# mako443/Text2Pos-CVPR2022

Measured on AMD Instinct MI355X. Metric: cells+queries encoded/sec and top-k retrieval QPS, 256-pt cells, 12k-cell DB, higher is better.
Workload: dtype f16x3 (fp32 operands split hi+lo into fp16, 3 f16 MFMAs, fp32 accumulate; fp32-class error) for the encoders / f64 MFMA for the ranking

## Files before the change

include/t2p.h:

```cpp
#ifndef T2P_H
#define T2P_H
#include <stddef.h>
#include <stdint.h>

#ifdef __cplusplus
extern "C" {
#endif

#define T2P_ABI_VERSION 29
#define T2P_DEFAULT_CHUNK_OBJECTS 65000
#define T2P_MAX_CHUNK_OBJECTS 65535
#define T2P_TUNING_MASK 0x1
#define T2P_E_ARG (-1)
#define T2P_E_WORKSPACE (-2)
#define T2P_E_UNSUPPORTED (-3)

typedef void* t2p_stream_t;

int t2p_abi_version(void);
const char* t2p_last_error(void);

typedef struct t2p_cell_weights {
    const float* sa_w1[3];
    const float* sa_b1[3];
    const float* sa_w2[3];
    const float* sa_b2[3];
    const float* ga_w1;
// ... 189 lines not shown
                               float* dx, t2p_stream_t stream);
int t2p_rownorm_backward(const float* x, const float* dy, int64_t n_rows, int32_t dim, float* dx, t2p_stream_t stream);

int t2p_pairwise_ranking(const float* scores, int32_t batch, float margin, float* row_loss, float* d_scores, float* row_count,
                         t2p_stream_t stream);

int t2p_hardest_ranking(const float* scores, int32_t batch, float margin, float* best, int32_t* where, float* d_scores,
                        t2p_stream_t stream);

int t2p_sample_group(const float* xyz, int64_t n_obj, int32_t n_pts, const float* radius_host ,
                     uint8_t* const* fps_idx , uint8_t* const* nbr , uint8_t* const* cnt ,
                     t2p_stream_t stream);
int t2p_group_rows(const float* xyz, int64_t n_obj, int32_t n_pts, const float* radius_host , int32_t self_loops,
                   uint8_t* const* fps_idx , uint16_t* const* rows , uint16_t* const* n_rows ,
                   t2p_stream_t stream);
int t2p_edge_counts(const uint16_t* rows, const uint16_t* n_rows, const int32_t* first_obj, int64_t n_obj, int32_t n_dense,
                    int32_t n_cent, int32_t self_loops, int32_t* counts, t2p_stream_t stream);
int t2p_edge_expand(const uint16_t* rows, const uint16_t* n_rows, const int32_t* first_obj, const int32_t* cent_ptr, int64_t n_obj,
                    int32_t n_dense, int32_t n_cent, int32_t self_loops, int32_t* src, int32_t* dst, t2p_stream_t stream);
int t2p_dedup_rows(const float* xyz, const float* rgb, int64_t n_obj, int32_t n_pts, uint16_t* rows, uint16_t* n_rows,
                   t2p_stream_t stream);
int t2p_knn(const float* x, int32_t dim, const int32_t* seg_ptr, int32_t n_seg, int32_t max_seg_rows, int32_t k,
            int32_t* out_idx, t2p_stream_t stream);
int t2p_gemm(const float* a, int32_t lda, const float* w, const float* bias, float* c, int32_t ldc, int32_t c0,
             int64_t m, int32_t k, int32_t n, int32_t relu, t2p_stream_t stream);
size_t t2p_gemm_tn_workspace_bytes(int64_t m, int32_t k1, int32_t n);
int t2p_gemm_tn(const float* a, int32_t lda, const float* b, int32_t ldb, float* c, int32_t ldc, int64_t m, int32_t k1, int32_t n,
                void* workspace, size_t workspace_bytes, t2p_stream_t stream);
size_t t2p_linear_wgrad_workspace_bytes(int64_t m, int32_t k1, int32_t n);
int t2p_linear_wgrad_f32(const float* dy, int32_t lda, const float* x, int32_t ldb, float* dw, int32_t ldc, float* colsum, int64_t m,
// ... 8 lines not shown
```

text2pos-cvpr2022_amd/_lib.py:

```python
import ctypes as C
import os

import torch

_HERE = os.path.dirname(os.path.abspath(__file__))
LIB_PATH = os.environ.get("T2P_LIB") or os.path.join(_HERE, "libt2p_hip.so")
ABI_VERSION = 29

c_float_p = C.POINTER(C.c_float)
c_void = C.c_void_p


class CellWeights(C.Structure):
    _names = (["sa_w1", "sa_b1", "sa_w2", "sa_b2"], ["ga_w1", "ga_b1", "ga_w2", "ga_b2", "lin1_w", "lin1_b", "lin2_w",
              "lin2_b", "pn_w", "pn_b", "col_w1", "col_b1", "col_w2", "col_b2", "pos_w1", "pos_b1", "pos_w2", "pos_b2",
              "merge_w", "merge_b", "g_wp", "g_bp", "g_wq", "g_w2", "g_b2", "lin_w1", "lin_b1", "lin_w2", "lin_b2"])
    _fields_ = ([(n, c_void * 3) for n in _names[0]] + [(n, c_void) for n in _names[1]] +
                [("sa_w2_x3", c_void * 3), ("ga_w2_x3", c_void), ("sa_b2_x3", c_void * 3), ("sa_w2_scale", C.c_float * 3),
                 ("lin1_x3", c_void), ("lin2_x3", c_void), ("merge_x3", c_void), ("pn_x3", c_void), ("g_wp_x3", c_void),
                 ("g_wq_x3", c_void), ("lin1_scale", C.c_float), ("lin2_scale", C.c_float), ("merge_scale", C.c_float),
                 ("pn_scale", C.c_float), ("g_wp_scale", C.c_float), ("g_wq_scale", C.c_float),
                 ("sa_w1_x3", c_void * 3), ("ga_w1_x3", c_void),
                 ("class_embedding", c_void), ("color_embedding", c_void),
                 ("ga_w1_l1", C.c_float), ("ga_b1_absmax", C.c_float), ("sa_wp_l1", C.c_float * 3),
# ... 73 lines not shown
    "t2p_pack_objects": (C.c_int, [c_void, c_void, c_void, c_void, c_void, C.c_int64, C.c_int32, c_void, c_void, c_void, c_void,
                                   c_void]),
    "t2p_pack_scene_objects": (C.c_int, [c_void, c_void, c_void, c_void, c_void, c_void, c_void, C.c_int64, C.c_int32, c_void, c_void,
                                         c_void, c_void, c_void, c_void]),
    "t2p_match_workspace_bytes": (C.c_size_t, [C.c_int64, C.c_int32, C.c_int32, C.c_int32]),
    "t2p_match": (C.c_int, [c_void, c_void, C.c_int64, C.c_int32, C.c_int32, C.c_int32, C.POINTER(MatchWeights),
                            C.c_int32, C.c_float, c_void, c_void, c_void, c_void, c_void, c_void, c_void, C.c_size_t,
                            c_void]),
    "t2p_profile_enable": (None, [C.c_int]),
    "t2p_profile_report": (C.c_int, [C.c_char_p, C.c_size_t]),
    "t2p_profile_repeat": (None, [C.c_char_p, C.c_int32]),
    "t2p_sample_group": (C.c_int, [c_void, C.c_int64, C.c_int32, c_float_p, C.POINTER(c_void), C.POINTER(c_void),
                                   C.POINTER(c_void), c_void]),
    "t2p_group_rows": (C.c_int, [c_void, C.c_int64, C.c_int32, c_float_p, C.c_int32, C.POINTER(c_void), C.POINTER(c_void),
                                 C.POINTER(c_void), c_void]),
    "t2p_edge_counts": (C.c_int, [c_void, c_void, c_void, C.c_int64, C.c_int32, C.c_int32, C.c_int32, c_void, c_void]),
    "t2p_edge_expand": (C.c_int, [c_void, c_void, c_void, c_void, C.c_int64, C.c_int32, C.c_int32, C.c_int32, c_void, c_void, c_void]),
    "t2p_dedup_rows": (C.c_int, [c_void, c_void, C.c_int64, C.c_int32, c_void, c_void, c_void]),
    "t2p_knn": (C.c_int, [c_void, C.c_int32, c_void, C.c_int32, C.c_int32, C.c_int32, c_void, c_void]),
    "t2p_gemm": (C.c_int, [c_void, C.c_int32, c_void, c_void, c_void, C.c_int32, C.c_int32, C.c_int64, C.c_int32,
                           C.c_int32, C.c_int32, c_void]),
    "t2p_rownorm": (C.c_int, [c_void, C.c_int64, C.c_int32, c_void, c_void]),
    "t2p_linear_wgrad_workspace_bytes": (C.c_size_t, [C.c_int64, C.c_int32, C.c_int32]),
    "t2p_linear_wgrad_f32": (C.c_int, [c_void, C.c_int32, c_void, C.c_int32, c_void, C.c_int32, c_void, C.c_int64, C.c_int32,
                                       C.c_int32, c_void, C.c_size_t, c_void]),
    "t2p_gemm_tn_workspace_bytes": (C.c_size_t, [C.c_int64, C.c_int32, C.c_int32]),
    "t2p_gemm_tn": (C.c_int, [c_void, C.c_int32, c_void, C.c_int32, c_void, C.c_int32, C.c_int64, C.c_int32, C.c_int32, c_void,
                              C.c_size_t, c_void]),
}

# ... 29 lines not shown
```

text2pos-cvpr2022_amd/csrc/api.hip:

```cpp
#include <stdarg.h>
#include <stdlib.h>
#include <string.h>

#include <mutex>
#include <set>
#include <utility>

#include "../../include/t2p.h"
#include "t2p_common.h"

namespace t2p {

static thread_local char g_err[512] = "";

void set_error(const char* fmt, ...) {
    va_list ap;
    va_start(ap, fmt);
    vsnprintf(g_err, sizeof(g_err), fmt, ap);
    va_end(ap);
}

int num_cus() {
    static int cached = 0;
    if (cached == 0) {
// ... 249 lines not shown
            gt.B[l] = lds_btab[l] ? nullptr : ws.B[l];
            gt.wp[l] = W.sa_w1[l] + (size_t)cf * Geo::H[l];
            gt.H[l] = Geo::H[l];
            gt.tail[l] = ws.F[l];
            gt.ld_tail[l] = Geo::LD[l];
            gt.tail_col0[l] = Geo::C[l];
        }
        gt.tail_rows[2] = g.gp;
        gt.A1 = sa1_points ? nullptr : ws.A[0];
        gt.w1 = W.sa_w1[0];
        gt.b1 = W.sa_b1[0];
        gt.rgb = rgb;
        gt.H1 = Geo::H[0];
        gt.guard = guard;

        T2P_TRY(launch_sample_group(xyz, n, cfg.n_pts, cfg.radius, gt, st));
        if (!(cfg.tuning & 1) && cfg.n_pts == 256)
            T2P_TRY(launch_dedup_rows(xyz, rgb, n, cfg.n_pts, gt.rows[0], gt.n_rows[0], g.nc[0], st));
        SaParams bp[3] = {};
        for (int l = 0; l < 3; l++) {
            bp[l].n_rows = gt.n_rows[l];
            bp[l].n_obj = n;
            bp[l].prefix_ws = ws.prefix[l];
            bp[l].bounds_ws = ws.bounds[l];
            bp[l].W_x3 = cfg.precision == 1 ? W.sa_w2_x3[l] : nullptr;
            bp[l].wp = lds_btab[l] ? W.sa_w1[l] : nullptr;
            bp[l].n_dense = g.nd[l];
            bp[l].n_cent = g.nc[l];
        }
        bp[0].w1 = sa1_points ? W.sa_w1[0] : nullptr;
        T2P_TRY(launch_sa_balance_levels(bp, Geo::H, Geo::C, st));
    }

    for (int l = 0; l < 3; l++) {
        const int H = Geo::H[l], C = Geo::C[l];
        const int cf = l == 0 ? 3 : Geo::C[l - 1];
        const float* pos_src = l == 0 ? xyz : ws.F[l - 1];
        const int ld_pos = l == 0 ? 3 : Geo::LD[l - 1];
        const int pos_col0 = l == 0 ? 0 : Geo::C[l - 1];
        if (l != 0) {
            WsParams p{};
            p.A = ws.F[l - 1];
            p.lda = Geo::LD[l - 1];
            p.k_live = Geo::C[l - 1] + 4;
            p.W = W.sa_w1[l];
// ... 678 lines not shown
    T2P_CHECK_ARG(xyz && radius_host && fps_idx && rows && n_rows, "group_rows: NULL argument");
    Geo g(n_pts);
    GroupTables gt{};
    gt.self_loops = self_loops ? 1 : 0;
    for (int l = 0; l < 3; l++) {
        T2P_CHECK_ARG(fps_idx[l] && rows[l] && n_rows[l], "group_rows: NULL table of level %d", l);
        gt.fps_idx[l] = fps_idx[l];
        gt.rows[l] = rows[l];
        gt.n_rows[l] = n_rows[l];
        gt.n_dense[l] = g.nd[l];
        gt.n_cent[l] = g.nc[l];
    }
    return launch_sample_group(xyz, n_obj, n_pts, radius_host, gt, (hipStream_t)stream);
}

int t2p_edge_counts(const uint16_t* rows, const uint16_t* n_rows, const int32_t* first_obj, int64_t n_obj, int32_t n_dense,
                    int32_t n_cent, int32_t self_loops, int32_t* counts, t2p_stream_t stream) {
    T2P_CHECK_ARG(n_obj >= 0 && (n_obj == 0 || (rows && n_rows && first_obj && counts)), "edge_counts: NULL argument");
    return launch_edge_counts(rows, n_rows, first_obj, n_obj, n_dense, n_cent, self_loops, counts, (hipStream_t)stream);
}

int t2p_edge_expand(const uint16_t* rows, const uint16_t* n_rows, const int32_t* first_obj, const int32_t* cent_ptr, int64_t n_obj,
                    int32_t n_dense, int32_t n_cent, int32_t self_loops, int32_t* src, int32_t* dst, t2p_stream_t stream) {
    T2P_CHECK_ARG(n_obj >= 0 && (n_obj == 0 || (rows && n_rows && first_obj && cent_ptr)), "edge_expand: NULL argument");
    return launch_edge_expand(rows, n_rows, first_obj, cent_ptr, n_obj, n_dense, n_cent, self_loops, src, dst, (hipStream_t)stream);
}

int t2p_pack_objects(const float* raw_xyz, const float* raw_rgb, const int32_t* obj_ptr, const int32_t* sample_idx,
                     const float* rot_cos_sin, int64_t n_obj, int32_t n_pts, float* xyz, float* rgb, float* center, float* mean_rgb,
                     t2p_stream_t stream) {
// ... 55 lines not shown
```

text2pos-cvpr2022_amd/csrc/sa_rows.hip:

```cpp
#ifndef T2P_RABL
#define T2P_RABL 0
#endif
#include "t2p_common.h"

namespace t2p {
int launch_sa_balance(const SaParams& p, int tile_rows, int n_wg, hipStream_t st);

namespace {

typedef _Float16 half8 __attribute__((ext_vector_type(8)));
typedef __fp16 fp16x2 __attribute__((ext_vector_type(2)));
typedef __attribute__((address_space(3))) void lds_void;
typedef const __attribute__((address_space(1))) void gl_void;

#define MFMA16(a, b, c) __builtin_amdgcn_mfma_f32_32x32x16_f16(a, b, c, 0, 0, 0)
#ifndef T2P_ROWS_AGPR
#define T2P_ROWS_AGPR 1
#endif
#ifndef T2P_ROWS_DIRECT
#define T2P_ROWS_DIRECT 1
#endif
__device__ __forceinline__ constexpr int rows_load_slot(int s, int c) {
    if (s == 0) return c == 0 || c == 4 ? -1 : 10 + (c < 4 ? c - 1 : c - 2);
    if (s == 1) return c == 1 ? 16 : (c == 3 ? 17 : -1);
// ... 31 lines not shown

template <int K, int N, int NC, int NW>
struct RowsCfg {
    static constexpr int NT = 64 * NW;
    static constexpr int ND = 2 * NC;
    static constexpr int S16 = K / 16, NTW = N / 32;
    static constexpr int SLOTS = K / 32;
    static constexpr int SLOT_BYTES = 32 * 128;
    static constexpr int RING_BYTES = SLOTS * SLOT_BYTES;
    static constexpr int MAXR = NC * 33;
    static constexpr int ROWS_CHUNKS = (MAXR * 2 + 1023) / 1024;
    static constexpr int ROWS_BUF = ROWS_CHUNKS * 1024;
    static constexpr int BT_STRIDE = K * 4 + 16;
    static constexpr int CPOS_BUF = 3 * NC * 4;
    static constexpr int ACC_OFF = 0;
    static constexpr int BT_OFF = ACC_OFF + NC * N * 4;
    static constexpr int ROWS_OFF = BT_OFF + NC * BT_STRIDE;
    static constexpr int CPOS_OFF = ROWS_OFF + 3 * ROWS_BUF;
    static constexpr int NR_OFF = CPOS_OFF + 2 * CPOS_BUF;
    static constexpr int SB_OFF = NR_OFF + kSubR * 2;
    static constexpr int DSTL_OFF = SB_OFF + kSubR * 4;
    static constexpr int RING_OFF = (DSTL_OFF + NW * 64 + 1023) / 1024 * 1024;
    static constexpr size_t lds_bytes() { return (size_t)RING_OFF + (T2P_ROWS_DIRECT ? (size_t)0 : (size_t)NW * RING_BYTES); }
    static_assert(K % 32 == 0 && N % 32 == 0 && NC % 64 == 0 && (NC * N / 4) % NT == 0, "shape");
    static_assert(SLOTS == 4, "the counted waits below assume four ring slots per tile (K = 128)");
};

template <int SEL>
__device__ __forceinline__ float sub_half_r(float v, fp16x2 h) {
    float r;
    if constexpr (SEL == 0)
        asm("v_fma_mix_f32 %0, %1, -1.0, %2 op_sel:[0,0,0] op_sel_hi:[1,0,0]" : "=v"(r) : "v"(h), "v"(v));
    else
        asm("v_fma_mix_f32 %0, %1, -1.0, %2 op_sel:[1,0,0] op_sel_hi:[1,0,0]" : "=v"(r) : "v"(h), "v"(v));
    return r;
}

__device__ __forceinline__ void lds_barrier_r() { asm volatile("s_waitcnt lgkmcnt(0)\n\ts_barrier" ::: "memory"); }
__device__ __forceinline__ void wait_ring() { asm volatile("s_waitcnt vmcnt(8)" ::: "memory"); }
__device__ __forceinline__ void wait_all_vm() { asm volatile("s_waitcnt vmcnt(0)" ::: "memory"); }
// ... 50 lines not shown

    uint32_t rd[2][2];
#pragma unroll
    for (int par = 0; par < 2; par++)
#pragma unroll
        for (int j = 0; j < 2; j++)
            rd[par][j] = ringb + (uint32_t)(rr * 128 + (((4 * par + 2 * h + j) ^ ((rr >> 1) & 7)) * 16));
    uint32_t dma_sel[4], dma_chunk[4];
#pragma unroll
    for (int q = 0; q < 4; q++) {
        const int r = 8 * q + (lane >> 3);
        dma_sel[q] = (uint32_t)(r * 4);
        dma_chunk[q] = (uint32_t)((((lane & 7) ^ ((r >> 1) & 7))) * 16);
    }

    for (int i = tid; i < NC * N; i += C::NT) acc_lds[i] = (int)0xFF800000;
    int gtop = 0;

    const int g_begin = p.bounds_ws[blockIdx.x], g_end = p.bounds_ws[blockIdx.x + 1];

    auto dma16 = [&](const void* base, uint32_t voff, uint32_t lds_off) {
        __builtin_amdgcn_global_load_lds((gl_void*)((const char*)base + voff), (lds_void*)(lds + lds_off), 16, 0, 0);
    };
    auto dma_rows = [&](int g) {
        const char* src = (const char*)(p.rows + (int64_t)g * C::MAXR);
        const uint32_t dst = (uint32_t)(C::ROWS_OFF + (g % 3) * C::ROWS_BUF);
#pragma unroll
        for (int c = 0; c < C::ROWS_CHUNKS; c++) {
            if (c % NW != wave) continue;
            uint32_t off = (uint32_t)(c * 1024 + lane * 16);
            if (off + 16 > (uint32_t)(C::MAXR * 2)) off = 0;
// ... 54 lines not shown
#pragma unroll
            for (int q = 0; q < 4; q++) dma_piece(voff, u, q);
        };
#if T2P_ROWS_DIRECT
        constexpr int AHEAD = 5;
        const uint32_t hoff = (uint32_t)(h * 32);
        auto load_half = [&](uint32_t roff, int s_, int j, f32x4 (&x)[2]) {
            if constexpr (!(T2P_RABL & 1)) x[j] = *(const f32x4*)((const char*)p.A + (size_t)roff + (size_t)(s_ * 64 + j * 16));
        };
        auto load_step = [&](uint32_t roff, int s_, f32x4 (&x)[2]) {
            load_half(roff, s_, 0, x);
            load_half(roff, s_, 1, x);
        };
#endif

        auto flush = [&](int g) {
            float* o = p.out + (int64_t)g * NC * (int64_t)p.ldo;
            int top = gtop;
            static_assert(C::NT % (N / 4) == 0, "a thread keeps its column quad over the drain");
#pragma unroll
            for (int k = 0; k < NC * N / 4 / C::NT; k++) {
                const int i = tid + k * C::NT;
                const int c = i / (N / 4), c4 = i % (N / 4);
                typedef int i32x4 __attribute__((ext_vector_type(4)));
                f32x4* a = (f32x4*)(acc_lds + c * N + c4 * 4);
                const f32x4 raw = *a;
                f32x4 v;
#pragma unroll
                for (int e = 0; e < 4; e++) {
                    const float r = fmaxf(raw[e] + bias4[e], 0.f);
                    const int bits = __float_as_int(r);
                    top = bits > top ? bits : top;
                    v[e] = r * p.out_scale;
                }
// ... 26 lines not shown
        lds_barrier_r();

        bool cur_fetched = false;
        uint32_t m_cur = 0;
#if T2P_ROWS_DIRECT
        uint32_t roff_cur = 0;
        f32x4 xw[C::S16][2];
#pragma unroll
        for (int s0 = 0; s0 < C::S16; s0++) xw[s0][0] = xw[s0][1] = f32x4{0.f, 0.f, 0.f, 0.f};
#endif

        for (int gi = 0; gi < cnt; gi++) {
            const int n_g = rows_of(gi), n_g1 = gi + 1 < cnt ? rows_of(gi + 1) : 0;
            const uint32_t sb_g = (uint32_t)__builtin_amdgcn_readfirstlane(sbase[gi]);
            const uint32_t sb_g1 = gi + 1 < cnt ? (uint32_t)__builtin_amdgcn_readfirstlane(sbase[gi + 1]) : 0u;
            int r0 = wave * 32;
            bool have = r0 < n_g;
            const bool did_tile = have;
            half8 a_hi, a_lo;
            f32x16 acc[C::NTW];
            bool pend = false;
            uint2 fourp[4] = {};
            auto read_step = [&](int s, uint32_t brow_, f32x4 (&x)[2], f32x4 (&b)[2]) {
#if T2P_ROWS_DIRECT
#pragma unroll
                for (int j = 0; j < 2; j++) {
                    x[j] = xw[s][j];
                    b[j] = *(const f32x4*)(lds + brow_ + s * 64 + j * 16);
                }
#else
// ... 31 lines not shown
                    m_cur = tile_meta(gi, r0, n_g);
#if T2P_ROWS_DIRECT
                    roff_cur = row_byte(gi, sb_g, m_cur) + hoff;
#pragma unroll
                    for (int s0 = 0; s0 < AHEAD; s0++) load_step(roff_cur, s0, xw[s0]);
#else
                    uint32_t v0[4];
                    tile_voff(row_byte(gi, sb_g, m_cur), v0);
#pragma unroll
                    for (int u = 0; u < C::SLOTS; u++) issue_slot(v0, u);
#endif
                }
                {
                    if constexpr (!T2P_ROWS_DIRECT) wait_ring();
                    f32x4 x[2], b[2];
                    read_step(0, (uint32_t)C::BT_OFF + ((m_cur >> 8) & 127u) * (uint32_t)C::BT_STRIDE + (uint32_t)(h * 32), x, b);
                    uint32_t nh[4], nl[4];
#pragma unroll
                    for (int pr = 0; pr < 4; pr++) {
                        float v[2];
                        prep_a(pr, x, b, v);
                        prep_b(v, nh[pr], nl[pr]);
                    }
                    a_hi = __builtin_bit_cast(half8, u32x4{nh[0], nh[1], nh[2], nh[3]});
                    a_lo = __builtin_bit_cast(half8, u32x4{nl[0], nl[1], nl[2], nl[3]});
                }
            }
            while (have) {
                const bool chain = r0 + NW * 32 < n_g;
                const bool nxt_ok = chain || (gi + 1 < cnt && wave * 32 < n_g1);
                const int gi_n = chain ? gi : (nxt_ok ? gi + 1 : gi);
                const int r0_n = chain ? r0 + NW * 32 : (nxt_ok ? wave * 32 : r0);
                const int n_n = (chain || !nxt_ok) ? n_g : n_g1;
                const uint32_t sb_n = (chain || !nxt_ok) ? sb_g : sb_g1;
                uint32_t m_nxt = tile_meta(gi_n, r0_n, n_n);
                uint32_t vn[4];
#if T2P_ROWS_DIRECT
                uint32_t roff_n = roff_cur;
                (void)vn;
#endif
                const uint32_t dl = (m_cur >> 8) & 127u;
                const uint32_t brow = (uint32_t)C::BT_OFF + dl * (uint32_t)C::BT_STRIDE + (uint32_t)(h * 32);
                asm volatile("ds_write_b16 %0, %1" ::"v"(dstl_addr + (uint32_t)(rr * 2)), "v"(dl * (uint32_t)(N * 4)) : "memory");
                uint2 four[4];

                uint32_t brow_n = 0;

#pragma unroll
                for (int s = 0; s < C::S16 - 1; s++) {
                    f32x4 x[2], b[2];
                    if (!T2P_ROWS_DIRECT && ((s + 1) & 1) == 0) wait_ring();
                    read_step(s + 1, brow, x, b);
                    if (s == C::S16 - 2) {
                        const uint32_t a4 = dstl_addr + (uint32_t)(h * 8);
                        asm volatile("ds_read_b64 %0, %4\n\tds_read_b64 %1, %4 offset:16\n\tds_read_b64 %2, %4 offset:32\n\t"
                                     "ds_read_b64 %3, %4 offset:48"
                                     : "=&v"(four[0]), "=&v"(four[1]), "=&v"(four[2]), "=&v"(four[3]) : "v"(a4) : "memory");
// ... 15 lines not shown
                    SB();
                    uint32_t nh[4], nl[4];
                    float v[2];
                    uint32_t rowbyte_n = 0;
#pragma unroll
                    for (int c = 0; c < 8; c++) {
                        if ((c & 1) == 0) prep_a(c >> 1, x, b, v);
                        else prep_b(v, nh[c >> 1], nl[c >> 1]);
                        if (s == 0) {
                            if (c == 2) rowbyte_n = row_byte(gi_n, sb_n, m_nxt);
#if T2P_ROWS_DIRECT
                            if (c == 4) roff_n = rowbyte_n + hoff;
#else
                            if (c == 4) tile_voff(rowbyte_n, vn);
#endif
                            if (c == 6) brow_n = (uint32_t)C::BT_OFF + ((m_nxt >> 8) & 127u) * (uint32_t)C::BT_STRIDE + (uint32_t)(h * 32);
                        }
#if T2P_ROWS_DIRECT
                        {
                            const int ld = rows_load_slot(s, c);
                            if (ld >= 0) load_half(ld < 2 * C::S16 ? roff_cur : roff_n, (ld >> 1) % C::S16, ld & 1, xw[(ld >> 1) % C::S16]);
                        }
#else
                        if ((s & 1) && (c & 1)) dma_piece(vn, s >> 1, c >> 1);
#endif
                        if (c < 4) mfma_w(acc[c], a_hi, w_lo[c][s], w_in_agpr(true, s), false);
                        else mfma_w(acc[c - 4], a_lo, w_hi[c - 4][s], w_in_agpr(false, s), false);
                        SB();
                    }
                    a_hi = __builtin_bit_cast(half8, u32x4{nh[0], nh[1], nh[2], nh[3]});
                    a_lo = __builtin_bit_cast(half8, u32x4{nl[0], nl[1], nl[2], nl[3]});
// ... 48 lines not shown
                            asm volatile(DS_MAX_STR ::"v"(ad[e]), "a"(acc[C::NTW - 1][e]), "n"((C::NTW - 1) * 128) : "memory");
                        pend = false;
                    }
                }
                have = chain;
                r0 = r0_n;
                cur_fetched = nxt_ok;
                m_cur = m_nxt;
#if T2P_ROWS_DIRECT
                roff_cur = roff_n;
#endif
            }
            if (!did_tile) cur_fetched = false;
            if (!did_tile) wait_all_vm();
            if constexpr (!(T2P_RABL & 16)) lds_barrier_r();
            if constexpr (!(T2P_RABL & 4)) flush(ga + gi);
            if (gi + 1 < cnt) {
                if constexpr (!(T2P_RABL & 4)) build_b(ga + gi + 1);
                if (gi + 3 < cnt) dma_rows(ga + gi + 3);
                if (gi + 2 < cnt) dma_cpos(ga + gi + 2);
            }
            if constexpr (!(T2P_RABL & 16)) lds_barrier_r();
        }
    }
    wait_all_vm();
    uint32_t gbits = 0;
    guard_track_bits(gbits, gtop);
    if (p.amax_out != nullptr && lane == 0 && gbits != 0u)
        atomicMax(p.amax_out, __float_as_uint(__uint_as_float(gbits) * p.out_scale));
}

// ... 39 lines not shown
```

text2pos-cvpr2022_amd/csrc/sample_group.hip:

```cpp
#include "t2p_common.h"

namespace t2p {

#pragma clang fp contract(off)

namespace {

#ifndef T2P_FPS_PK
#define T2P_FPS_PK 1
#endif

constexpr int kMaxPts = 256;
constexpr int kMaxNbr = 32;

__device__ __forceinline__ float dist2(float ax, float ay, float az, float bx, float by, float bz) {
#pragma clang fp contract(off)
    float dx = ax - bx, dy = ay - by, dz = az - bz;
    float xx = dx * dx, yy = dy * dy, zz = dz * dz;
    float s = xx + yy;
    return s + zz;
}

template <int CTRL>
__device__ __forceinline__ int dpp_i(int v) {
// ... 93 lines not shown
            if (nbr_lds) cnt_lds[c] = (uint8_t)kept;
            if (self_loops && rows_out) rows_out[base + kept] = (uint16_t)(((c | 0x80) << 8) | c);
        }
        base += kept + (self_loops ? 1 : 0);
        if (c + 1 < n_c) {
            const float mx = wave_max_f(bd);
            const unsigned long long tie = __ballot(bd == mx);
            cur = __builtin_amdgcn_readlane(bi, (int)__builtin_ctzll(tie));
        }
    }
    if (rows_out && lane < 4 && base + lane < n_c * (kMaxNbr + 1)) rows_out[base + lane] = 0xFFFF;
    *n_rows_out = base;
    __syncthreads();
}

template <int PPL>
__device__ void level_fast(const float* px, const float* py, const float* pz, int n_c, float r2, uint8_t* sel, float* qx,
                           float* qy, float* qz, uint16_t* __restrict__ rows_out, int self_loops, int* n_rows_out) {
    const int lane = threadIdx.x;
    const int i0 = lane * PPL;
    float x[PPL], y[PPL], z[PPL];
    uint32_t mind[PPL];
#pragma unroll
    for (int j = 0; j < PPL; j++) {
        x[j] = px[i0 + j];
        y[j] = py[i0 + j];
        z[j] = pz[i0 + j];
        mind[j] = 0x7f800000u;
    }
    int cur = 0;
    int base = 0;
    for (int c = 0; c < n_c; c++) {
        const float cx = px[cur], cy = py[cur], cz = pz[cur];
        if (lane == 0) {
            sel[c] = (uint8_t)cur;
            qx[c] = cx;
            qy[c] = cy;
            qz[c] = cz;
        }
        float d[PPL];
        unsigned long long m[PPL];
        if constexpr (T2P_FPS_PK && PPL % 2 == 0) {
            typedef float f32x2 __attribute__((ext_vector_type(2)));
            const f32x2 c2x = {cx, cx}, c2y = {cy, cy}, c2z = {cz, cz};
#pragma unroll
            for (int j = 0; j < PPL; j += 2) {
#pragma clang fp contract(off)
                const f32x2 dx = f32x2{x[j], x[j + 1]} - c2x, dy = f32x2{y[j], y[j + 1]} - c2y, dz = f32x2{z[j], z[j + 1]} - c2z;
                const f32x2 xx = dx * dx, yy = dy * dy, zz = dz * dz;
                const f32x2 sxy = xx + yy;
                const f32x2 dd = sxy + zz;
                d[j] = dd[0];
                d[j + 1] = dd[1];
// ... 5 lines not shown
            }
        } else {
#pragma unroll
            for (int j = 0; j < PPL; j++) {
                d[j] = dist2(x[j], y[j], z[j], cx, cy, cz);
                mind[j] = min(mind[j], __float_as_uint(d[j]));
                m[j] = __ballot(d[j] < r2);
            }
        }
        int lower = 0, count = 0;
#pragma unroll
        for (int j = 0; j < PPL; j++) {
            lower = __builtin_amdgcn_mbcnt_hi((uint32_t)(m[j] >> 32), __builtin_amdgcn_mbcnt_lo((uint32_t)m[j], lower));
            count += __popcll(m[j]);
        }
        const uint32_t tag = (uint32_t)c << 8;
        char* const rows_b = (char*)rows_out;
        if (count <= kMaxNbr) {
            uint32_t off = 2u * (uint32_t)(base + lower);
#pragma unroll
            for (int j = 0; j < PPL; j++) {
                const bool hit = d[j] < r2;
                if (hit) *(uint16_t*)(rows_b + off) = (uint16_t)(tag | (uint32_t)(i0 + j));
                off += hit ? 2u : 0u;
            }
        } else {
            uint32_t pos = (uint32_t)lower;
#pragma unroll
            for (int j = 0; j < PPL; j++) {
                const bool hit = d[j] < r2;
                if (hit && pos < (uint32_t)kMaxNbr) *(uint16_t*)(rows_b + 2u * ((uint32_t)base + pos)) = (uint16_t)(tag | (uint32_t)(i0 + j));
// ... 125 lines not shown
                            {p3, p3 + kMaxPts / 8, p3 + kMaxPts / 4}};
        const float rr[3] = {r0 * r0, r1 * r1, r2 * r2};
#pragma unroll
        for (int l = 0; l < 3; l++) {
            const int n_d = gt.n_dense[l], n_c = gt.n_cent[l];
            if (want_nbr) {
                for (int i = lane; i < n_c * kMaxNbr / 4; i += 64) ((uint32_t*)nbr_lds)[i] = 0u;
            }
            __syncthreads();
            int n_rows = 0;
            uint16_t* g_rows16 = gt.rows[l] ? gt.rows[l] + o * (int64_t)(n_c * (kMaxNbr + 1)) : nullptr;
            if constexpr (FAST) {
                if (l == 0)
                    level_fast<4>(pin[l][0], pin[l][1], pin[l][2], n_c, rr[l], sel_lds, pin[l + 1][0], pin[l + 1][1],
                                  pin[l + 1][2], g_rows16, gt.self_loops, &n_rows);
                else if (l == 1)
                    level_fast<2>(pin[l][0], pin[l][1], pin[l][2], n_c, rr[l], sel_lds, pin[l + 1][0], pin[l + 1][1],
                                  pin[l + 1][2], g_rows16, gt.self_loops, &n_rows);
                else
                    level_fast<1>(pin[l][0], pin[l][1], pin[l][2], n_c, rr[l], sel_lds, pin[l + 1][0], pin[l + 1][1],
                                  pin[l + 1][2], g_rows16, gt.self_loops, &n_rows);
            } else if (n_d > 128)
                level<4>(pin[l][0], pin[l][1], pin[l][2], n_d, n_c, rr[l], sel_lds, pin[l + 1][0], pin[l + 1][1],
                         pin[l + 1][2], nbr_lds, cnt_lds, g_rows16, gt.self_loops, &n_rows);
            else if (n_d > 64)
                level<2>(pin[l][0], pin[l][1], pin[l][2], n_d, n_c, rr[l], sel_lds, pin[l + 1][0], pin[l + 1][1],
                         pin[l + 1][2], nbr_lds, cnt_lds, g_rows16, gt.self_loops, &n_rows);
            else
                level<1>(pin[l][0], pin[l][1], pin[l][2], n_d, n_c, rr[l], sel_lds, pin[l + 1][0], pin[l + 1][1],
                         pin[l + 1][2], nbr_lds, cnt_lds, g_rows16, gt.self_loops, &n_rows);
// ... 149 lines not shown
```

text2pos-cvpr2022_amd/csrc/t2p_common.h:

```cpp
#pragma once
#include <hip/hip_runtime.h>
#include <stdint.h>
#include <stdio.h>

namespace t2p {

void set_error(const char* fmt, ...);

#define T2P_E_ARG (-1)
#define T2P_E_WORKSPACE (-2)
#define T2P_E_UNSUPPORTED (-3)

#define T2P_CHECK_ARG(cond, ...)                  \
    do {                                          \
        if (!(cond)) {                            \
            ::t2p::set_error(__VA_ARGS__);        \
            return T2P_E_ARG;                     \
        }                                         \
    } while (0)

#define T2P_CHECK_LAUNCH(name)                                                   \
    do {                                                                         \
        hipError_t e__ = hipGetLastError();                                      \
        if (e__ != hipSuccess) {                                                 \
// ... 100 lines not shown
    ~ProfScope();
    int slot;
    hipStream_t st;
    void* ev_end;
    int reps;
};
#define T2P_REPEAT(ps) for (int rep_ = (ps).reps; rep_ > 0; --rep_)

struct GroupTables {
    uint8_t* fps_idx[3];
    uint8_t* nbr[3];
    uint8_t* cnt[3];
    uint16_t* rows[3];
    uint16_t* n_rows[3];
    int self_loops;
    int n_dense[3];
    int n_cent[3];
    float* B[3];
    const float* wp[3];
    int H[3];
    float* tail[3];
    int ld_tail[3], tail_col0[3];
    int tail_rows[3];
    float* A1;
    const float* w1;
    const float* b1;
    const float* rgb;
    int H1;
    uint32_t* guard;
};
// ... 90 lines not shown
    int ld_pos, pos_col0;
    const float* feat_src;
    const float* w1;
    const float* b1;
    int n_dense, n_cent;
    int64_t n_obj;
    int32_t* prefix_ws;
    int32_t* bounds_ws;
    int balanced;
    uint32_t* amax_out;
    int out_rows;
};
int launch_ws_sa(int H, int C, const SaParams& p, hipStream_t st);
int launch_sa_x3(int H, int C, const SaParams& p, hipStream_t st);
int sa_x3_launch_shape(int H, int C, int64_t n_obj, int* tile_rows, int* n_wg);
bool sa_rows_selected(int H, int C, const SaParams& p);
int launch_sa_rows(int H, int C, const SaParams& p, hipStream_t st);
int sa_rows_launch_shape(int64_t n_obj, int* tile_rows, int* n_wg);
bool sa_points_selected(int H, int C, const SaParams& p);
int launch_sa_points(int H, int C, const SaParams& p, hipStream_t st);
int sa_points_launch_shape(int64_t n_obj, int* tile_rows, int* n_wg);
bool sa3_selected(int H, int C, const SaParams& p);
int launch_sa3(const SaParams& p, hipStream_t st);
int sa3_launch_shape(int64_t n_obj, int* tile_rows, int* n_wg);
int launch_sa_balance_levels(const SaParams p[3], const int H[3], const int C[3], hipStream_t st);

int launch_bilstm_impl(const float* gate_table , const float* whh ,
                       const void* whh_x3 ,
                       float whh_scale, const int32_t* tokens , const int32_t* lengths, int B, int T, int V, int D,
                       float* hdir_ws , float* out ,
                       hipStream_t st);

int launch_lstm_cell_fwd(const float* pre, const float* table, const int32_t* tokens, const int32_t* lengths, int64_t B, int T,
                         int D, int step, int reverse, const float* c_prev, const float* h_prev, float* gates, float* c,
                         float* h, hipStream_t st);
int launch_lstm_cell_bwd(const float* dh_gemm, const float* dh_carry_in, const float* dc_in, const float* gates,
                         const float* c_prev, const float* c, const int32_t* lengths, int64_t B, int D, int step, float* d_pre,
                         float* dc_out, float* dh_carry_out, hipStream_t st);

// ... 31 lines not shown
```

text2pos-cvpr2022_amd/ops.py:

```python
import ctypes as C
import os
from typing import Dict, Optional

import numpy as np
import torch

from . import _lib as L

_workspaces: Dict[tuple, torch.Tensor] = {}


def _stream(device) -> C.c_void_p:
    return C.c_void_p(torch.cuda.current_stream(device).cuda_stream)


def _ptr(t: Optional[torch.Tensor]) -> C.c_void_p:
    return C.c_void_p(0 if t is None else t.data_ptr())


def _need(t: torch.Tensor, name: str, dtype, ndim=None, device=None):
    if not isinstance(t, torch.Tensor):
        raise RuntimeError(f"{name}: expected a torch.Tensor, got {type(t).__name__}")
    if not t.is_cuda:
        raise RuntimeError(f"{name}: must live on the GPU (got device {t.device}); there is no CPU path")
# ... 159 lines not shown
        counts = torch.empty((n_obj * ncs[l],), dtype=torch.int32, device=dev)
        L.check(L.lib().t2p_edge_counts(_ptr(rows[l]), _ptr(n_rows[l]), _ptr(first_obj), n_obj, nds[l], ncs[l],
                                        int(bool(self_loops)), _ptr(counts), st), "t2p_edge_counts")
        cp = torch.zeros((n_obj * ncs[l] + 1,), dtype=torch.int32, device=dev)
        torch.cumsum(counts, 0, dtype=torch.int32, out=cp[1:])
        cent_ptrs.append(cp)
    totals = torch.stack([cp[-1] for cp in cent_ptrs]).cpu().tolist()
    out = []
    for l in range(3):
        e = int(totals[l])
        src = torch.empty((e,), dtype=torch.int32, device=dev)
        dst = torch.empty((e,), dtype=torch.int32, device=dev)
        L.check(L.lib().t2p_edge_expand(_ptr(rows[l]), _ptr(n_rows[l]), _ptr(first_obj), _ptr(cent_ptrs[l]), n_obj, nds[l], ncs[l],
                                        int(bool(self_loops)), _ptr(src), _ptr(dst), st), "t2p_edge_expand")
        out.append(dict(fps_idx=fps[l], src=src, dst=dst, cent_ptr=cent_ptrs[l], n_dense=nds[l], n_cent=ncs[l]))
    return out


def dedup_rows(xyz: torch.Tensor, rgb: torch.Tensor, rows: torch.Tensor, n_rows: torch.Tensor):
    _need(xyz, "xyz", torch.float32, 3)
    _need(rgb, "rgb", torch.float32, 3, xyz.device)
    _need(rows, "rows", torch.int16, 2, xyz.device)
    _need(n_rows, "n_rows", torch.int16, 1, xyz.device)
    n_obj, n_pts = xyz.shape[0], xyz.shape[1]
    if rows.shape[0] != n_obj or rows.shape[1] != ((n_pts + 1) // 2) * 33 or n_rows.numel() != n_obj:
        raise RuntimeError("dedup_rows: inconsistent shapes")
    L.check(L.lib().t2p_dedup_rows(_ptr(xyz), _ptr(rgb), n_obj, n_pts, _ptr(rows), _ptr(n_rows), _stream(xyz.device)),
            "t2p_dedup_rows")


# ... 564 lines not shown
```

Baseline: 154,100.

## Share neighbour rows of repeated FPS tail centroids at SA level 2

Once farthest-point sampling runs out of distinct points, it keeps returning index 0. At SA level 2 the grouping now writes that repeated tail centroid's neighbour rows only once, under a shared slot code. The row-GEMM kernel max-reduces those rows into an extra accumulator row, then broadcasts it into every tail centroid at flush time, so duplicate neighbour rows are no longer computed. This adds one LDS accumulator row and a ballot-and-merge step to each flush, and it only applies to 256-point objects when the rows kernel is selected.

```diff
diff --git a/include/t2p.h b/include/t2p.h
--- a/include/t2p.h
+++ b/include/t2p.h
@@ -7,10 +7,10 @@
 extern "C" {
 #endif
 
-#define T2P_ABI_VERSION 29
+#define T2P_ABI_VERSION 30
 #define T2P_DEFAULT_CHUNK_OBJECTS 65000
 #define T2P_MAX_CHUNK_OBJECTS 65535
-#define T2P_TUNING_MASK 0x1
+#define T2P_TUNING_MASK 0x5
 #define T2P_E_ARG (-1)
 #define T2P_E_WORKSPACE (-2)
 #define T2P_E_UNSUPPORTED (-3)
@@ -230,6 +230,9 @@
 int t2p_group_rows(const float* xyz, int64_t n_obj, int32_t n_pts, const float* radius_host , int32_t self_loops,
                    uint8_t* const* fps_idx , uint16_t* const* rows , uint16_t* const* n_rows ,
                    t2p_stream_t stream);
+int t2p_group_rows_shared(const float* xyz, int64_t n_obj, int32_t n_pts, const float* radius_host , int32_t self_loops,
+                          int32_t share_mask, uint8_t* const* fps_idx , uint16_t* const* rows ,
+                          uint16_t* const* n_rows , t2p_stream_t stream);
 int t2p_edge_counts(const uint16_t* rows, const uint16_t* n_rows, const int32_t* first_obj, int64_t n_obj, int32_t n_dense,
                     int32_t n_cent, int32_t self_loops, int32_t* counts, t2p_stream_t stream);
 int t2p_edge_expand(const uint16_t* rows, const uint16_t* n_rows, const int32_t* first_obj, const int32_t* cent_ptr, int64_t n_obj,
diff --git a/profiles/tail_rows_census.py b/profiles/tail_rows_census.py
--- /dev/null
+++ b/profiles/tail_rows_census.py
@@ -0,0 +1,89 @@
+#!/usr/bin/env python
+import argparse
+import os
+import sys
+
+import numpy as np
+
+sys.path.insert(0, os.path.join(os.path.dirname(os.path.abspath(__file__)), ".."))
+
+RADII = (0.2, 0.3, 0.4)
+MAX_NBR = 32
+
+
+def level(pos: np.ndarray, r: float):
+    n_d = pos.shape[0]
+    n_c = (n_d + 1) // 2
+    r2 = np.float32(r) * np.float32(r)
+    mind = np.full(n_d, np.inf, dtype=np.float32)
+    fps = np.zeros(n_c, dtype=np.int64)
+    cnt = np.zeros(n_c, dtype=np.int64)
+    cur = 0
+    for c in range(n_c):
+        fps[c] = cur
+        d = pos - pos[cur]
+        d2 = (d[:, 0] * d[:, 0] + d[:, 1] * d[:, 1]) + d[:, 2] * d[:, 2]
+        cnt[c] = min(int((d2 < r2).sum()), MAX_NBR)
+        mind = np.minimum(mind, d2)
+        cur = int(np.argmax(mind))
+    return fps, cnt
+
+
+def dedup_hits(pos: np.ndarray, rgb: np.ndarray, fps: np.ndarray, r: float) -> int:
+    key = np.concatenate([pos, rgb], axis=1).view(np.uint32)
+    _, first = np.unique(key, axis=0, return_index=True)
+    orig = np.zeros(pos.shape[0], dtype=bool)
+    orig[first] = True
+    r2 = np.float32(r) * np.float32(r)
+    kept = 0
+    for c in fps:
+        d = pos - pos[c]
+        d2 = (d[:, 0] * d[:, 0] + d[:, 1] * d[:, 1]) + d[:, 2] * d[:, 2]
+        hits = np.flatnonzero(d2 < r2)[:MAX_NBR]
+        kept += int(orig[hits].sum())
+    return kept
+
+
+def main():
+    ap = argparse.ArgumentParser(description=__doc__.split("\n")[0])
+    ap.add_argument("--seed", type=int, default=20220002, help="bench.py's object stream")
+    ap.add_argument("--objects", type=int, default=3000)
+    args = ap.parse_args()
+    from importlib import import_module
+    S = import_module("text2pos-cvpr2022_amd.synthetic")
+    xyz, rgb, _, _ = S.make_objects(args.seed, 0, args.objects)
+    n = xyz.shape[0]
+    rows = np.zeros(3)
+    rows_dedup = 0.0
+    with_tail = np.zeros(3)
+    tail_cent = np.zeros(3)
+    tail_rows = np.zeros(3)
+    executed = np.zeros(3)
+    cents = np.zeros(3)
+    for o in range(n):
+        pos = xyz[o].astype(np.float32)
+        for l in range(3):
+            fps, cnt = level(pos, RADII[l])
+            n_c = fps.shape[0]
+            tail = (fps == 0) & (np.arange(n_c) > 0)
+            all_rows = cnt.sum() + n_c
+            t_rows = cnt[tail].sum()
+            rows[l] += all_rows
+            cents[l] += n_c
+            with_tail[l] += tail.any()
+            tail_cent[l] += tail.sum()
+            tail_rows[l] += t_rows
+            executed[l] += all_rows - t_rows + (cnt[0] if tail.any() else 0)
+            if l == 0:
+                rows_dedup += dedup_hits(pos, rgb[o].astype(np.float32), fps, RADII[0]) + n_c
+            pos = pos[fps]
+    print(f"{n} objects of seed {args.seed}")
+    print("level | rows/object | objects with a tail | tail centroids | tail rows (non-self) | rows/object, tail shared")
+    for l in range(3):
+        extra = f" ({rows_dedup / n:.0f} after point dedup)" if l == 0 else ""
+        print(f"SA{l + 1}   | {rows[l] / n:8.0f}{extra} | {100 * with_tail[l] / n:5.1f} % | {100 * tail_cent[l] / cents[l]:5.1f} % | "
+              f"{100 * tail_rows[l] / rows[l]:5.1f} % | {executed[l] / n:8.0f} ({100 * (executed[l] / rows[l] - 1):+.1f} %)")
+
+
+if __name__ == "__main__":
+    main()
diff --git a/text2pos-cvpr2022_amd/_lib.py b/text2pos-cvpr2022_amd/_lib.py
--- a/text2pos-cvpr2022_amd/_lib.py
+++ b/text2pos-cvpr2022_amd/_lib.py
@@ -5,7 +5,7 @@
 
 _HERE = os.path.dirname(os.path.abspath(__file__))
 LIB_PATH = os.environ.get("T2P_LIB") or os.path.join(_HERE, "libt2p_hip.so")
-ABI_VERSION = 29
+ABI_VERSION = 30
 
 c_float_p = C.POINTER(C.c_float)
 c_void = C.c_void_p
@@ -111,6 +111,8 @@
                                    C.POINTER(c_void), c_void]),
     "t2p_group_rows": (C.c_int, [c_void, C.c_int64, C.c_int32, c_float_p, C.c_int32, C.POINTER(c_void), C.POINTER(c_void),
                                  C.POINTER(c_void), c_void]),
+    "t2p_group_rows_shared": (C.c_int, [c_void, C.c_int64, C.c_int32, c_float_p, C.c_int32, C.c_int32, C.POINTER(c_void),
+                                        C.POINTER(c_void), C.POINTER(c_void), c_void]),
     "t2p_edge_counts": (C.c_int, [c_void, c_void, c_void, C.c_int64, C.c_int32, C.c_int32, C.c_int32, c_void, c_void]),
     "t2p_edge_expand": (C.c_int, [c_void, c_void, c_void, c_void, C.c_int64, C.c_int32, C.c_int32, C.c_int32, c_void, c_void, c_void]),
     "t2p_dedup_rows": (C.c_int, [c_void, c_void, C.c_int64, C.c_int32, c_void, c_void, c_void]),
diff --git a/text2pos-cvpr2022_amd/csrc/api.hip b/text2pos-cvpr2022_amd/csrc/api.hip
--- a/text2pos-cvpr2022_amd/csrc/api.hip
+++ b/text2pos-cvpr2022_amd/csrc/api.hip
@@ -287,9 +287,6 @@
         gt.H1 = Geo::H[0];
         gt.guard = guard;
 
-        T2P_TRY(launch_sample_group(xyz, n, cfg.n_pts, cfg.radius, gt, st));
-        if (!(cfg.tuning & 1) && cfg.n_pts == 256)
-            T2P_TRY(launch_dedup_rows(xyz, rgb, n, cfg.n_pts, gt.rows[0], gt.n_rows[0], g.nc[0], st));
         SaParams bp[3] = {};
         for (int l = 0; l < 3; l++) {
             bp[l].n_rows = gt.n_rows[l];
@@ -302,6 +299,11 @@
             bp[l].n_cent = g.nc[l];
         }
         bp[0].w1 = sa1_points ? W.sa_w1[0] : nullptr;
+        for (int l = 0; l < 3; l++) gt.share_tail[l] = sa_shares_tail_rows(l, Geo::H[l], Geo::C[l], bp[l], cfg.n_pts, cfg.tuning) ? 1 : 0;
+
+        T2P_TRY(launch_sample_group(xyz, n, cfg.n_pts, cfg.radius, gt, st));
+        if (!(cfg.tuning & 1) && cfg.n_pts == 256)
+            T2P_TRY(launch_dedup_rows(xyz, rgb, n, cfg.n_pts, gt.rows[0], gt.n_rows[0], g.nc[0], st));
         T2P_TRY(launch_sa_balance_levels(bp, Geo::H, Geo::C, st));
     }
 
@@ -1010,6 +1012,27 @@
     return launch_sample_group(xyz, n_obj, n_pts, radius_host, gt, (hipStream_t)stream);
 }
 
+int t2p_group_rows_shared(const float* xyz, int64_t n_obj, int32_t n_pts, const float* radius_host, int32_t self_loops,
+                          int32_t share_mask, uint8_t* const* fps_idx, uint16_t* const* rows, uint16_t* const* n_rows,
+                          t2p_stream_t stream) {
+    T2P_CHECK_ARG(xyz && radius_host && fps_idx && rows && n_rows, "group_rows_shared: NULL argument");
+    T2P_CHECK_ARG((share_mask & ~2) == 0, "group_rows_shared: share_mask=%#x (bit 1: SA level 2; no other level has a shared form)", share_mask);
+    T2P_CHECK_ARG(share_mask == 0 || n_pts == 256, "group_rows_shared: shared lists exist for 256 points per object (n_pts = %d)", n_pts);
+    Geo g(n_pts);
+    GroupTables gt{};
+    gt.self_loops = self_loops ? 1 : 0;
+    for (int l = 0; l < 3; l++) {
+        T2P_CHECK_ARG(fps_idx[l] && rows[l] && n_rows[l], "group_rows_shared: NULL table of level %d", l);
+        gt.fps_idx[l] = fps_idx[l];
+        gt.rows[l] = rows[l];
+        gt.n_rows[l] = n_rows[l];
+        gt.n_dense[l] = g.nd[l];
+        gt.n_cent[l] = g.nc[l];
+        gt.share_tail[l] = (share_mask >> l) & 1;
+    }
+    return launch_sample_group(xyz, n_obj, n_pts, radius_host, gt, (hipStream_t)stream);
+}
+
 int t2p_edge_counts(const uint16_t* rows, const uint16_t* n_rows, const int32_t* first_obj, int64_t n_obj, int32_t n_dense,
                     int32_t n_cent, int32_t self_loops, int32_t* counts, t2p_stream_t stream) {
     T2P_CHECK_ARG(n_obj >= 0 && (n_obj == 0 || (rows && n_rows && first_obj && counts)), "edge_counts: NULL argument");
diff --git a/text2pos-cvpr2022_amd/csrc/sa_rows.hip b/text2pos-cvpr2022_amd/csrc/sa_rows.hip
--- a/text2pos-cvpr2022_amd/csrc/sa_rows.hip
+++ b/text2pos-cvpr2022_amd/csrc/sa_rows.hip
@@ -69,7 +69,8 @@
     static constexpr int BT_STRIDE = K * 4 + 16;
     static constexpr int CPOS_BUF = 3 * NC * 4;
     static constexpr int ACC_OFF = 0;
-    static constexpr int BT_OFF = ACC_OFF + NC * N * 4;
+    static constexpr int XROW = kSaTailCode;
+    static constexpr int BT_OFF = ACC_OFF + (NC + 1) * N * 4;
     static constexpr int ROWS_OFF = BT_OFF + NC * BT_STRIDE;
     static constexpr int CPOS_OFF = ROWS_OFF + 3 * ROWS_BUF;
     static constexpr int NR_OFF = CPOS_OFF + 2 * CPOS_BUF;
@@ -79,6 +80,7 @@
     static constexpr size_t lds_bytes() { return (size_t)RING_OFF + (T2P_ROWS_DIRECT ? (size_t)0 : (size_t)NW * RING_BYTES); }
     static_assert(K % 32 == 0 && N % 32 == 0 && NC % 64 == 0 && (NC * N / 4) % NT == 0, "shape");
     static_assert(SLOTS == 4, "the counted waits below assume four ring slots per tile (K = 128)");
+    static_assert(XROW == NC && (NC & (NC - 1)) == 0 && XROW * N * 4 <= 0xFFFF && XROW < 128, "shared tail slot");
 };
 
 template <int SEL>
@@ -159,7 +161,7 @@
         dma_chunk[q] = (uint32_t)((((lane & 7) ^ ((r >> 1) & 7))) * 16);
     }
 
-    for (int i = tid; i < NC * N; i += C::NT) acc_lds[i] = (int)0xFF800000;
+    for (int i = tid; i < (NC + 1) * N; i += C::NT) acc_lds[i] = (int)0xFF800000;
     int gtop = 0;
 
     const int g_begin = p.bounds_ws[blockIdx.x], g_end = p.bounds_ws[blockIdx.x + 1];
@@ -244,10 +246,26 @@
         };
 #endif
 
-        auto flush = [&](int g) {
+        auto flush = [&](int g, int t0) {
             float* o = p.out + (int64_t)g * NC * (int64_t)p.ldo;
             int top = gtop;
             static_assert(C::NT % (N / 4) == 0, "a thread keeps its column quad over the drain");
+            if (t0 < NC) {
+                f32x4* const ax = (f32x4*)(acc_lds + C::XROW * N + (tid % (N / 4)) * 4);
+                const f32x4 xq = *ax;
+#pragma unroll 1
+                for (int c = tid / (N / 4); c < NC; c += C::NT / (N / 4)) {
+                    if (c < t0) continue;
+                    f32x4* a = (f32x4*)(acc_lds + c * N + (tid % (N / 4)) * 4);
+                    f32x4 r = *a;
+#pragma unroll
+                    for (int e = 0; e < 4; e++) r[e] = fmaxf(r[e], xq[e]);
+                    *a = r;
+                }
+                lds_barrier_r();
+                typedef int i32x4 __attribute__((ext_vector_type(4)));
+                if (tid < N / 4) *(i32x4*)ax = i32x4{(int)0xFF800000, (int)0xFF800000, (int)0xFF800000, (int)0xFF800000};
+            }
 #pragma unroll
             for (int k = 0; k < NC * N / 4 / C::NT; k++) {
                 const int i = tid + k * C::NT;
@@ -304,6 +322,14 @@
             const int n_g = rows_of(gi), n_g1 = gi + 1 < cnt ? rows_of(gi + 1) : 0;
             const uint32_t sb_g = (uint32_t)__builtin_amdgcn_readfirstlane(sbase[gi]);
             const uint32_t sb_g1 = gi + 1 < cnt ? (uint32_t)__builtin_amdgcn_readfirstlane(sbase[gi + 1]) : 0u;
+            int t0;
+            {
+                static_assert(NC == 64, "one lane per centroid");
+                const uint32_t* cp = (const uint32_t*)(lds + C::CPOS_OFF + ((ga + gi) & 1) * C::CPOS_BUF);
+                const bool same = lane > 0 && cp[lane] == cp[0] && cp[NC + lane] == cp[NC] && cp[2 * NC + lane] == cp[2 * NC];
+                const unsigned long long tm = __ballot(same);
+                t0 = tm ? (int)__builtin_ctzll(tm) : NC;
+            }
             int r0 = wave * 32;
             bool have = r0 < n_g;
             const bool did_tile = have;
@@ -365,7 +391,7 @@
                 {
                     if constexpr (!T2P_ROWS_DIRECT) wait_ring();
                     f32x4 x[2], b[2];
-                    read_step(0, (uint32_t)C::BT_OFF + ((m_cur >> 8) & 127u) * (uint32_t)C::BT_STRIDE + (uint32_t)(h * 32), x, b);
+                    read_step(0, (uint32_t)C::BT_OFF + ((m_cur >> 8) & (uint32_t)(NC - 1)) * (uint32_t)C::BT_STRIDE + (uint32_t)(h * 32), x, b);
                     uint32_t nh[4], nl[4];
 #pragma unroll
                     for (int pr = 0; pr < 4; pr++) {
@@ -391,7 +417,7 @@
                 (void)vn;
 #endif
                 const uint32_t dl = (m_cur >> 8) & 127u;
-                const uint32_t brow = (uint32_t)C::BT_OFF + dl * (uint32_t)C::BT_STRIDE + (uint32_t)(h * 32);
+                const uint32_t brow = (uint32_t)C::BT_OFF + (dl & (uint32_t)(NC - 1)) * (uint32_t)C::BT_STRIDE + (uint32_t)(h * 32);
                 asm volatile("ds_write_b16 %0, %1" ::"v"(dstl_addr + (uint32_t)(rr * 2)), "v"(dl * (uint32_t)(N * 4)) : "memory");
                 uint2 four[4];
 
@@ -437,7 +463,7 @@
 #else
                             if (c == 4) tile_voff(rowbyte_n, vn);
 #endif
-                            if (c == 6) brow_n = (uint32_t)C::BT_OFF + ((m_nxt >> 8) & 127u) * (uint32_t)C::BT_STRIDE + (uint32_t)(h * 32);
+                            if (c == 6) brow_n = (uint32_t)C::BT_OFF + ((m_nxt >> 8) & (uint32_t)(NC - 1)) * (uint32_t)C::BT_STRIDE + (uint32_t)(h * 32);
                         }
 #if T2P_ROWS_DIRECT
                         {
@@ -516,7 +542,7 @@
             if (!did_tile) cur_fetched = false;
             if (!did_tile) wait_all_vm();
             if constexpr (!(T2P_RABL & 16)) lds_barrier_r();
-            if constexpr (!(T2P_RABL & 4)) flush(ga + gi);
+            if constexpr (!(T2P_RABL & 4)) flush(ga + gi, t0);
             if (gi + 1 < cnt) {
                 if constexpr (!(T2P_RABL & 4)) build_b(ga + gi + 1);
                 if (gi + 3 < cnt) dma_rows(ga + gi + 3);
diff --git a/text2pos-cvpr2022_amd/csrc/sample_group.hip b/text2pos-cvpr2022_amd/csrc/sample_group.hip
--- a/text2pos-cvpr2022_amd/csrc/sample_group.hip
+++ b/text2pos-cvpr2022_amd/csrc/sample_group.hip
@@ -131,9 +131,10 @@
     __syncthreads();
 }
 
-template <int PPL>
+template <int PPL, bool SHARE = false>
 __device__ void level_fast(const float* px, const float* py, const float* pz, int n_c, float r2, uint8_t* sel, float* qx,
-                           float* qy, float* qz, uint16_t* __restrict__ rows_out, int self_loops, int* n_rows_out) {
+                           float* qy, float* qz, uint16_t* __restrict__ rows_out, int self_loops, int* n_rows_out,
+                           int tail_code = 0) {
     const int lane = threadIdx.x;
     const int i0 = lane * PPL;
     float x[PPL], y[PPL], z[PPL];
@@ -147,6 +148,7 @@
     }
     int cur = 0;
     int base = 0;
+    [[maybe_unused]] bool tail_open = false;
     for (int c = 0; c < n_c; c++) {
         const float cx = px[cur], cy = py[cur], cz = pz[cur];
         if (lane == 0) {
@@ -154,6 +156,16 @@
             qx[c] = cx;
             qy[c] = cy;
             qz[c] = cz;
+        }
+        bool tail = false;
+        if constexpr (SHARE) {
+            tail = c > 0 && cur == 0;
+            if (tail && tail_open) {
+                if (self_loops && lane == 0) rows_out[(uint32_t)base] = (uint16_t)(((c | 0x80) << 8) | c);
+                base += self_loops ? 1 : 0;
+                continue;
+            }
+            tail_open = tail;
         }
         float d[PPL];
         unsigned long long m[PPL];
@@ -189,7 +201,7 @@
             lower = __builtin_amdgcn_mbcnt_hi((uint32_t)(m[j] >> 32), __builtin_amdgcn_mbcnt_lo((uint32_t)m[j], lower));
             count += __popcll(m[j]);
         }
-        const uint32_t tag = (uint32_t)c << 8;
+        const uint32_t tag = (uint32_t)(tail ? tail_code : c) << 8;
         char* const rows_b = (char*)rows_out;
         if (count <= kMaxNbr) {
             uint32_t off = 2u * (uint32_t)(base + lower);
@@ -345,6 +357,9 @@
                 if (l == 0)
                     level_fast<4>(pin[l][0], pin[l][1], pin[l][2], n_c, rr[l], sel_lds, pin[l + 1][0], pin[l + 1][1],
                                   pin[l + 1][2], g_rows16, gt.self_loops, &n_rows);
+                else if (l == 1 && gt.share_tail[1])
+                    level_fast<2, true>(pin[l][0], pin[l][1], pin[l][2], n_c, rr[l], sel_lds, pin[l + 1][0], pin[l + 1][1],
+                                        pin[l + 1][2], g_rows16, gt.self_loops, &n_rows, kSaTailCode);
                 else if (l == 1)
                     level_fast<2>(pin[l][0], pin[l][1], pin[l][2], n_c, rr[l], sel_lds, pin[l + 1][0], pin[l + 1][1],
                                   pin[l + 1][2], g_rows16, gt.self_loops, &n_rows);
diff --git a/text2pos-cvpr2022_amd/csrc/t2p_common.h b/text2pos-cvpr2022_amd/csrc/t2p_common.h
--- a/text2pos-cvpr2022_amd/csrc/t2p_common.h
+++ b/text2pos-cvpr2022_amd/csrc/t2p_common.h
@@ -138,6 +138,7 @@
     uint16_t* rows[3];
     uint16_t* n_rows[3];
     int self_loops;
+    int share_tail[3];
     int n_dense[3];
     int n_cent[3];
     float* B[3];
@@ -258,6 +259,7 @@
 int launch_ws_sa(int H, int C, const SaParams& p, hipStream_t st);
 int launch_sa_x3(int H, int C, const SaParams& p, hipStream_t st);
 int sa_x3_launch_shape(int H, int C, int64_t n_obj, int* tile_rows, int* n_wg);
+constexpr int kSaTailCode = 64;
 bool sa_rows_selected(int H, int C, const SaParams& p);
 int launch_sa_rows(int H, int C, const SaParams& p, hipStream_t st);
 int sa_rows_launch_shape(int64_t n_obj, int* tile_rows, int* n_wg);
@@ -267,6 +269,9 @@
 bool sa3_selected(int H, int C, const SaParams& p);
 int launch_sa3(const SaParams& p, hipStream_t st);
 int sa3_launch_shape(int64_t n_obj, int* tile_rows, int* n_wg);
+inline bool sa_shares_tail_rows(int l, int H, int C, const SaParams& p, int n_pts, int tuning) {
+    return l == 1 && n_pts == 256 && !(tuning & 4) && p.n_dense == 128 && p.n_cent == 64 && sa_rows_selected(H, C, p);
+}
 int launch_sa_balance_levels(const SaParams p[3], const int H[3], const int C[3], hipStream_t st);
 
 int launch_bilstm_impl(const float* gate_table , const float* whh ,
diff --git a/text2pos-cvpr2022_amd/ops.py b/text2pos-cvpr2022_amd/ops.py
--- a/text2pos-cvpr2022_amd/ops.py
+++ b/text2pos-cvpr2022_amd/ops.py
@@ -197,6 +197,26 @@
         L.check(L.lib().t2p_edge_expand(_ptr(rows[l]), _ptr(n_rows[l]), _ptr(first_obj), _ptr(cent_ptrs[l]), n_obj, nds[l], ncs[l],
                                         int(bool(self_loops)), _ptr(src), _ptr(dst), st), "t2p_edge_expand")
         out.append(dict(fps_idx=fps[l], src=src, dst=dst, cent_ptr=cent_ptrs[l], n_dense=nds[l], n_cent=ncs[l]))
+    return out
+
+
+def group_rows(xyz: torch.Tensor, radius=(0.2, 0.3, 0.4), self_loops: bool = True, share_mask: int = 0):
+    _need(xyz, "xyz", torch.float32, 3)
+    dev = xyz.device
+    n_obj, n_pts, three = xyz.shape
+    if three != 3:
+        raise RuntimeError(f"xyz: last dimension must be 3, got {three}")
+    nd, out = n_pts, dict(fps_idx=[], rows=[], n_rows=[])
+    for _ in range(3):
+        nc = (nd + 1) // 2
+        out["fps_idx"].append(torch.empty((n_obj, nc), dtype=torch.uint8, device=dev))
+        out["rows"].append(torch.empty((n_obj, nc * 33), dtype=torch.int16, device=dev))
+        out["n_rows"].append(torch.empty((n_obj,), dtype=torch.int16, device=dev))
+        nd = nc
+    arr = lambda ts: (C.c_void_p * 3)(*[t.data_ptr() for t in ts])
+    r = (C.c_float * 3)(*[float(v) for v in radius])
+    L.check(L.lib().t2p_group_rows_shared(_ptr(xyz), n_obj, n_pts, r, int(bool(self_loops)), int(share_mask), arr(out["fps_idx"]),
+                                          arr(out["rows"]), arr(out["n_rows"]), _stream(dev)), "t2p_group_rows_shared")
     return out
 
 
```

Measured after the change: 156,900, median of 6. 1.02x the previous value.
